# NVlabs/intrinsic3d

Hardware: AMD Instinct MI355X
Metric: Gauss-Newton iterations/s at the finest SDF level (higher is better)
Workload: dtype f32

## Files before the change

include/intrinsic3d_hip.h:

```cpp
#ifndef INTRINSIC3D_HIP_H
#define INTRINSIC3D_HIP_H
#include <stdint.h>
#ifdef __cplusplus
extern "C" {
#endif

typedef struct i3d_context i3d_context;

typedef enum {
    I3D_OK = 0,
    I3D_ERR_INVALID_ARGUMENT = 1,
    I3D_ERR_NO_DEVICE = 2,
    I3D_ERR_HIP = 3,
    I3D_ERR_STATE = 4,
    I3D_ERR_CAPACITY = 5,
    I3D_ERR_COMM = 6,
    I3D_ERR_IO = 7
} i3d_status;

int  i3d_create(int32_t device_ordinal, i3d_context** out);
void i3d_destroy(i3d_context* ctx);
const char* i3d_last_error(const i3d_context* ctx);
const char* i3d_version(void);

// ... 222 lines not shown
int i3d_timing_get_work_ex(i3d_context* ctx, double* ms, int64_t* launches, double* slow_ms , int64_t* slow_launches );
const char* i3d_kernel_name(int32_t k);
int i3d_problem_sizes(i3d_context* ctx, int64_t out[6]);

int i3d_debug_assemble(i3d_context* ctx, const i3d_optimizer_config* cfg, int32_t iteration, int32_t* slots_out);
int64_t i3d_debug_map_order(const int32_t* keys, int64_t n, int32_t mode, int32_t* order);
int i3d_debug_flags(i3d_context* ctx, uint8_t* flags );
int i3d_debug_eg_rows(i3d_context* ctx, int32_t* frame , float* weight ,
                      float* residual , float* jac );
int i3d_debug_reg_rows(i3d_context* ctx, uint8_t* has_er , uint8_t* has_es , float* ea_weight );
int i3d_debug_neighbors(i3d_context* ctx, int32_t* nbr );
int i3d_debug_normal_eq(i3d_context* ctx, double* gradient, double* jtj_diag, double* cost);
int i3d_debug_jtj_apply(i3d_context* ctx, const double* x, double* y);
int i3d_debug_counters(i3d_context* ctx, int64_t* stream_syncs);
int i3d_debug_ladder_stats(i3d_context* ctx, int64_t* out6);
int i3d_debug_cull_stats(i3d_context* ctx, int64_t* pairs, int64_t* culled);

#ifdef __cplusplus
}
#endif
#endif
```

intrinsic3d_amd/binding.py:

```python
from __future__ import annotations

import ctypes as C
import os

import numpy as np

_HERE = os.path.dirname(os.path.abspath(__file__))
LIB_PATH = os.environ.get("I3D_LIB") or os.path.join(_HERE, "libintrinsic3d_hip.so")

K_NAMES = ["classify", "observe", "build", "eg_pass", "gather", "cost", "vector", "sh", "eg_aux", "comm", "eg_mr2", "eg_mr3"]


class OptimizerConfig(C.Structure):
    _fields_ = [("iterations", C.c_int32), ("lm_steps", C.c_int32),
                ("lambda_g", C.c_double), ("lambda_r0", C.c_double), ("lambda_r1", C.c_double),
                ("lambda_s0", C.c_double), ("lambda_s1", C.c_double), ("lambda_a", C.c_double),
                ("fix_poses", C.c_int32), ("fix_intrinsics", C.c_int32), ("fix_distortion", C.c_int32),
                ("occlusion_distance", C.c_float), ("num_observations", C.c_int32),
                ("thres_shell", C.c_double), ("grid_level", C.c_int32), ("rgbd_level", C.c_int32),
                ("pcg_fixed_iterations", C.c_int32), ("verbose", C.c_int32), ("carry_trust_radius", C.c_int32), ("fix_sdf", C.c_int32)]


class IterationStats(C.Structure):
    _fields_ = [("rows", C.c_int64 * 4), ("weight_sum", C.c_double * 4), ("type_weight", C.c_double * 4),
# ... 77 lines not shown
           "i3d_set_frames", "i3d_set_frames_rgbd", "i3d_get_frame_image", "i3d_resize_depth", "i3d_set_camera", "i3d_get_camera", "i3d_set_voxel_sh", "i3d_get_voxel_sh",
           "i3d_optimizer_config_default", "i3d_optimize", "i3d_optimize_host", "i3d_estimate_sh",
           "i3d_set_grid_from_tsdf_records", "i3d_recompute_colors", "i3d_clear_outside_thin_shell", "i3d_upsample", "i3d_grid_info",
           "i3d_export_grid", "i3d_refine",
           "i3d_tsdf_read_header", "i3d_tsdf_read_records", "i3d_tsdf_write", "i3d_sbr_write", "i3d_sbr_read", "i3d_write_poses",
           "i3d_write_intrinsics", "i3d_read_intrinsics", "i3d_config_load_yaml", "i3d_yaml_get",
           "i3d_extract_mesh", "i3d_get_mesh", "i3d_render_view", "i3d_track_desc_default", "i3d_track_frame", "i3d_export_mesh_ply", "i3d_write_ply", "i3d_mc_tables", "i3d_visualization_colors",
           "i3d_png_info", "i3d_png_decode", "i3d_pose_mat_to_vec6", "i3d_sensor_open", "i3d_sensor_open_yaml", "i3d_sensor_close", "i3d_sensor_info", "i3d_sensor_color",
           "i3d_sensor_depth", "i3d_sensor_pose", "i3d_sensor_set_pose", "i3d_sensor_set_pose_vec6", "i3d_sensor_save_poses",
           "i3d_mesh_remove_loose_components", "i3d_keyframes_load", "i3d_keyframes_save", "i3d_keyframes_select", "i3d_blur_score", "i3d_init_frames_from_sensor",
           "i3d_fusion_create", "i3d_fusion_destroy", "i3d_fusion_last_error", "i3d_fusion_integrate", "i3d_fusion_finish", "i3d_fusion_info", "i3d_fusion_get",
           "i3d_fusion_save", "i3d_fusion_render", "i3d_fusion_track", "i3d_shard_need", "i3d_comm_stats",
           "i3d_comm_unique_id", "i3d_comm_init", "i3d_comm_sim_create", "i3d_comm_sim_destroy", "i3d_comm_init_sim", "i3d_shard_plan", "i3d_shard_vec_index",
           "i3d_comm_transport", "i3d_timing_enable", "i3d_timing_select", "i3d_timing_get", "i3d_timing_get_work", "i3d_timing_get_work_ex", "i3d_kernel_name", "i3d_problem_sizes",
           "i3d_debug_assemble", "i3d_debug_map_order", "i3d_debug_flags", "i3d_debug_eg_rows", "i3d_debug_reg_rows", "i3d_debug_neighbors",
           "i3d_debug_normal_eq", "i3d_debug_jtj_apply", "i3d_debug_counters", "i3d_debug_cull_stats", "i3d_debug_ladder_stats", "i3d_debug_track_sums"]

_lib = None


def load():
    global _lib
    if _lib is not None:
        return _lib
    if not os.path.exists(LIB_PATH):
        raise RuntimeError(f"{LIB_PATH} is missing: build it with `make -C intrinsic3d_amd/csrc` "
                           "(or __graft_entry__.build()); the product path has no CPU fallback")
    L = C.CDLL(LIB_PATH)
    vp, i32, i64, f32, f64 = C.c_void_p, C.c_int32, C.c_int64, C.c_float, C.c_double
    L.i3d_create.restype = i32; L.i3d_create.argtypes = [i32, C.POINTER(vp)]
    L.i3d_destroy.argtypes = [vp]
# ... 30 lines not shown
    L.i3d_timing_get.restype = i32; L.i3d_timing_get.argtypes = [vp, vp, vp, i32]
    L.i3d_timing_get_work.restype = i32; L.i3d_timing_get_work.argtypes = [vp, vp, vp]
    L.i3d_timing_get_work_ex.restype = i32; L.i3d_timing_get_work_ex.argtypes = [vp, vp, vp, vp, vp]
    L.i3d_kernel_name.restype = C.c_char_p; L.i3d_kernel_name.argtypes = [i32]
    L.i3d_comm_transport.restype = C.c_char_p; L.i3d_comm_transport.argtypes = [vp]
    L.i3d_problem_sizes.restype = i32; L.i3d_problem_sizes.argtypes = [vp, vp]
    L.i3d_debug_assemble.restype = i32; L.i3d_debug_assemble.argtypes = [vp, C.POINTER(OptimizerConfig), i32, C.POINTER(i32)]
    L.i3d_debug_flags.restype = i32; L.i3d_debug_flags.argtypes = [vp, vp]
    L.i3d_debug_eg_rows.restype = i32; L.i3d_debug_eg_rows.argtypes = [vp, vp, vp, vp, vp]
    L.i3d_debug_reg_rows.restype = i32; L.i3d_debug_reg_rows.argtypes = [vp, vp, vp, vp]
    L.i3d_debug_neighbors.restype = i32; L.i3d_debug_neighbors.argtypes = [vp, vp]
    L.i3d_debug_normal_eq.restype = i32; L.i3d_debug_normal_eq.argtypes = [vp, vp, vp, C.POINTER(f64)]
    L.i3d_debug_jtj_apply.restype = i32; L.i3d_debug_jtj_apply.argtypes = [vp, vp, vp]
    L.i3d_debug_counters.restype = i32; L.i3d_debug_counters.argtypes = [vp, vp]
    L.i3d_debug_ladder_stats.restype = i32; L.i3d_debug_ladder_stats.argtypes = [vp, vp]
    L.i3d_debug_cull_stats.restype = i32; L.i3d_debug_cull_stats.argtypes = [vp, vp, vp]
    L.i3d_set_grid_from_tsdf_records.restype = i32; L.i3d_set_grid_from_tsdf_records.argtypes = [vp, f32, i64, vp, vp, vp, vp]
    L.i3d_recompute_colors.restype = i32; L.i3d_recompute_colors.argtypes = [vp, f32, i32]
    L.i3d_clear_outside_thin_shell.restype = i32; L.i3d_clear_outside_thin_shell.argtypes = [vp, f64, C.POINTER(i64)]
    L.i3d_upsample.restype = i32; L.i3d_upsample.argtypes = [vp, C.POINTER(i64)]
    L.i3d_grid_info.restype = i32; L.i3d_grid_info.argtypes = [vp, C.POINTER(i64), C.POINTER(f32), C.POINTER(f32)]
    L.i3d_export_grid.restype = i32; L.i3d_export_grid.argtypes = [vp, vp, vp, vp, vp, vp, vp]
    L.i3d_refine.restype = i32; L.i3d_refine.argtypes = [vp, C.POINTER(RefineConfig), C.POINTER(OptimizerConfig), REFINE_CALLBACK, vp]
    u64 = C.c_uint64; cp = C.c_char_p
    L.i3d_tsdf_read_header.restype = i32; L.i3d_tsdf_read_header.argtypes = [cp, C.POINTER(f32), C.POINTER(f32), C.POINTER(f32), C.POINTER(u64), C.POINTER(f32)]
    L.i3d_tsdf_read_records.restype = i32; L.i3d_tsdf_read_records.argtypes = [cp, u64, vp, vp, vp, vp]
    L.i3d_tsdf_write.restype = i32; L.i3d_tsdf_write.argtypes = [cp, f32, f32, f32, f32, u64, vp, vp, vp, vp]
    L.i3d_sbr_write.restype = i32; L.i3d_sbr_write.argtypes = [cp, f32, f32, f32, f32, u64, vp, vp, vp, vp, vp, vp]
    L.i3d_sbr_read.restype = i32; L.i3d_sbr_read.argtypes = [cp, u64, vp, vp, vp, vp, vp, vp]
    L.i3d_write_poses.restype = i32; L.i3d_write_poses.argtypes = [cp, i32, vp, vp]
# ... 354 lines not shown
        NP = 2 * self.N + 6 * self.K + 9
        g = np.zeros(NP); d = np.zeros(NP); cost = C.c_double(0)
        self._check(self.L.i3d_debug_normal_eq(self.h, _p(g), _p(d), C.byref(cost)), "i3d_debug_normal_eq")
        return g, d, cost.value

    def debug_counters(self):
        n = C.c_int64(0)
        self._check(self.L.i3d_debug_counters(self.h, C.byref(n)), "i3d_debug_counters")
        return {"stream_syncs": int(n.value)}

    def debug_ladder_stats(self):
        a = (C.c_int64 * 6)()
        self._check(self.L.i3d_debug_ladder_stats(self.h, a), "i3d_debug_ladder_stats")
        return {"batches": int(a[0]), "row_streams": int(a[1]), "system_passes": int(a[2]), "resyncs": int(a[3]), "unused_systems": int(a[4]), "depth": int(a[5])}

    def debug_cull_stats(self):
        a = C.c_int64(0); b = C.c_int64(0)
        self._check(self.L.i3d_debug_cull_stats(self.h, C.byref(a), C.byref(b)), "i3d_debug_cull_stats")
        return int(a.value), int(b.value)

    def debug_jtj_apply(self, x):
        x = np.ascontiguousarray(x, np.float64); y = np.zeros_like(x)
        self._check(self.L.i3d_debug_jtj_apply(self.h, _p(x), _p(y)), "i3d_debug_jtj_apply")
        return y


def shard_need(A, world, anbr, active):
    anbr = np.ascontiguousarray(anbr, np.int32); active = np.ascontiguousarray(active, np.uint8); need = np.zeros(A, np.uint64)
    rc = load().i3d_shard_need(int(A), int(world), _p(anbr), _p(active), _p(need))
    if rc != 0:
# ... 329 lines not shown
```

intrinsic3d_amd/csrc/device/kernels.hpp:

```cpp
#pragma once
#include "common.hpp"
#include "p2p_device.hpp"

namespace i3d {

struct HashTable { unsigned long long* keys; int* vals; unsigned int mask; };
void launch_sort_keys(hipStream_t st, int N, const int* keys_xyz , unsigned long long* sort_keys, int* iota);
void launch_permute_grid(hipStream_t st, int N, const int* perm, const int* keys_xyz, const double* sdf, const double* sdf_ref,
                         const double* alb, const float* w, const uint8_t* rgb,
                         int* cx, int* cy, int* cz, int* rank, double* sdf0, double* x_sdf, double* x_alb, float* f_sdf, float* f_alb,
                         float* weight, uchar4* color);
void launch_hash_build(hipStream_t st, int N, const int* cx, const int* cy, const int* cz, HashTable t);
void launch_nbr_build(hipStream_t st, int N, const int* cx, const int* cy, const int* cz, HashTable t, int* nbr);
void launch_classify(hipStream_t st, GridView g, OptParams p, int* active_flag);
void launch_compact(hipStream_t st, int N, const int* active_flag, const int* active_scan, const uint8_t* flags, int* aidx, int* alist, uint8_t* aflags);
void launch_partition_blocks(hipStream_t st, GridView g, int A, int* alist, uint8_t* aflags, int* aidx);
void launch_group_rows(hipStream_t st, int A, const uint8_t* nrows, int* gmax);
void launch_anbr(hipStream_t st, int N, int A, int Acap, const int* alist, const int* nbr, const int* aidx, int* anbr);
void launch_scatter_sh(hipStream_t st, int N, const int* rank, const double* sh_visit , float* sh );
void launch_gather_visit(hipStream_t st, int N, const int* rank, const double* x_sdf, const double* x_alb, double* out_sdf, double* out_alb);
void launch_update_fields(hipStream_t st, int N, const int* rank, const double* sdf_ref, const double* alb, const uint8_t* rgb,
                          double* x_sdf, double* x_alb, float* f_sdf, float* f_alb, uchar4* color);

void launch_observe(hipStream_t st, GridView g, RowView r, OptParams p, const FrameConst* frames, const unsigned* cull_mask = nullptr, bool prefilter = false);
// ... 81 lines not shown
int    tile_plan_hmax();
inline int tile_plan_hmax_of(int T) { return T == 1024 ? 2048 : 1536; }
inline int tile_plan_tiles_of(int A, int T) { return (A + T - 1) / T; }
size_t tile_plan_temp_bytes(int ntiles);
hipError_t launch_tile_plan(hipStream_t st, RowView r, TilePlan t, void* temp, size_t temp_bytes);
void launch_eaw_sym(hipStream_t st, RowView r, TilePlan t, const int* cflag );
int  launch_eg_tile(hipStream_t st, RowView r, OptParams p, const float* u, TilePlan t, double* shared, float* qacc, double* pq_partials ,
                    const PcgState* state, float* cam_partials = nullptr, int cam_stride = 0);
void launch_ext_offsets(hipStream_t st, int n, const int* ext_e, int A, int* ext_off);
void eg_tile_launch_shape(const TilePlan& t, int K, int& blocks, int& tiles_per_block);

struct LadVec;
int  eg_tile_mr_max_systems(int K);
int  launch_eg_tile_mr(hipStream_t st, RowView r, OptParams p, TilePlan t, int nsys, const int* sys, const float* u0, float* qacc0, float* qh0, double* pq0 , float* cam0, int cam_stride,
                       const PcgState* st0 , const LadVec& lv);

struct ShardArgs {
    P2PDev pd; RimLists rim; int seq;
    int n_slice_partials;
    int n_rim_wg;
    const float* zb; float* pb; float* ub; const float* cmb; int chunk;
};
struct LadVec {
    size_t vec;
    size_t qh;
    size_t cam;
    size_t part;
    size_t mblk;
    size_t tail;
    int sysid[LADDER_MAX];
// ... 59 lines not shown
```

intrinsic3d_amd/csrc/device/tile_pass_mr.hip:

```cpp
#include <cstring>
#include <algorithm>
#include <vector>
#include <cstdlib>
#include "kernels.hpp"
#include "reduce_device.hpp"
#include "wave_ops.hpp"
#include "tile_device.hpp"

namespace i3d {

constexpr int MR_T = 512, MR_HMAX = 1536, MR_NWV = MR_T / 64, MR_TC = 32;

template <int NB> struct MrConst {
    static constexpr int T = MR_T, HMAX = MR_HMAX, NW = MR_NWV, TC = MR_TC, NSLOT = T + HMAX + 1;
    static constexpr int CAMW = (NW * 9 + 3) & ~3, VSTR = NW * TC * 6;
    static constexpr int O_U = 0, UB = (2 * NSLOT + 3) & ~3;
    static constexpr int O_TR = O_U + NB * UB, TRB = (T + 4 + 3) & ~3;
    static constexpr int D_FLAG = O_TR + NB * TRB, D_CAM9W = D_FLAG + 4, D_TAG = D_CAM9W + NB * CAMW, D_VAL = D_TAG + NW * TC;
    static constexpr int O_LIST = D_VAL + NB * VSTR, O_C = O_LIST + 2 * HMAX, O_OFFS = O_C + 12 * T, O_PQ = O_OFFS + (((HMAX + 4) / 2 + 3) & ~3), D0 = O_PQ + NB * 2 * T;
};
struct MrLayout { int o_upose, o_ui, SK; size_t bytes; };
static __host__ __device__ inline MrLayout mr_layout(int D0, int NB, int K) {
    const int rs = (6 * K) | 1;
    MrLayout L;
    L.o_upose = (rs + 9 + 3) & ~3; L.o_ui = (L.o_upose + 6 * K + 3) & ~3; L.SK = L.o_ui + 12;
// ... 61 lines not shown
constexpr int MR_NPH = 12;
__device__ unsigned long long g_mr_phase[3][MR_NPH + 2];
#define PH_DECL unsigned long long ph_[MR_NPH] = {0, 0, 0, 0, 0, 0, 0, 0, 0, 0, 0, 0}; unsigned long long ph_t_ = __builtin_amdgcn_s_memtime(); unsigned ph_tiles_ = 0
#define PH(k) do { const unsigned long long t_ = __builtin_amdgcn_s_memtime(); ph_[k] += t_ - ph_t_; ph_t_ = t_; } while (0)
#define PH_TILE ++ph_tiles_
#define PH_FLUSH(NBv) do { if ((threadIdx.x & 63u) == 0u) { for (int k_ = 0; k_ < MR_NPH; ++k_) atomicAdd(&g_mr_phase[(NBv) - 1][k_], ph_[k_]); atomicAdd(&g_mr_phase[(NBv) - 1][MR_NPH], (unsigned long long)ph_tiles_); atomicAdd(&g_mr_phase[(NBv) - 1][MR_NPH + 1], 1ull); } } while (0)
#else
#define PH_DECL
#define PH(k)
#define PH_TILE
#define PH_FLUSH(NBv)
#endif
#ifdef I3D_MR_BLOCKTIME
__device__ unsigned long long g_mr_blk[3][1024], g_mr_blk_n[3][1024];
#define BT_DECL const unsigned long long bt0_ = __builtin_amdgcn_s_memtime()
#define BT_FLUSH(NBv) do { if (threadIdx.x == 0u && blockIdx.x < 1024u) { atomicAdd(&g_mr_blk[(NBv) - 1][blockIdx.x], __builtin_amdgcn_s_memtime() - bt0_); atomicAdd(&g_mr_blk_n[(NBv) - 1][blockIdx.x], 1ull); } } while (0)
#else
#define BT_DECL
#define BT_FLUSH(NBv)
#endif

struct MrArgs {
    const float* u0; float* qacc0; float* qh0; double* pq0 ; float* cam0;
    const PcgState* st0;
    size_t vec, qh, cam, part;
    int sys[3];
};

template <int NB, bool GHOSTS>
__global__ void __launch_bounds__(MR_T, 2) k_eg_tile_mr(RowView r, OptParams p, MrArgs m, const unsigned* __restrict__ lnbr, const float* __restrict__ eaw_sym, const int* __restrict__ halo_idx,
                                                        const int* __restrict__ halo_cnt, int tiles_per_block, int ntl, int cam_stride, const int* __restrict__ gmaxv,
                                                        const unsigned short* __restrict__ hp_off, const unsigned short* __restrict__ hp_src,
                                                        int tile_first, int n_own, const int* __restrict__ ghost_list) {
    constexpr int T = MR_T, HMAX = MR_HMAX, NW = MR_NWV, TC = MR_TC, ZSLOT = T + HMAX, NCOL = 12, HPCAP = 4 * HMAX, NQH = HMAX / T;
    bool alive[NB];
    {
        bool any = false;
#pragma unroll
        for (int b = 0; b < NB; ++b) { alive[b] = m.st0[2 * m.sys[b]].done == 0; any = any || alive[b]; }
        if (!any) return;
    }
    extern __shared__ float lds[];
    const int K = p.K; const size_t Acap = r.Acap; const int A = r.A, chunk = r.chunk;
    const int nshared = 6 * K + 9, rs = (6 * K) | 1;
    using MC = MrConst<NB>;
    constexpr int D_FLAG = MC::D_FLAG, D_CAM9W = MC::D_CAM9W, CAMW = MC::CAMW, D_TAG = MC::D_TAG, D_VAL = MC::D_VAL, D0 = MC::D0;
    const MrLayout L = mr_layout(D0, NB, K);
    const int SB = L.SK, o_upose = L.o_upose, o_ui = L.o_ui;
#define SYS(b) (D0 + (b) * SB)
#define U_S(b) (MC::O_U + (b) * MC::UB)
#define U_A(b) (MC::O_U + (b) * MC::UB + MC::NSLOT)
#define TR_L(b) (MC::O_TR + (b) * MC::TRB)
#define C_L (MC::O_C)
#define hp_list reinterpret_cast<unsigned short*>(lds + MC::O_LIST)
// ... 7 lines not shown
        for (int e = i; e < rs + 9; e += T) lds[SYS(b) + e] = 0.0f;
        for (int e = i; e < 6 * K; e += T) lds[SYS(b) + o_upose + e] = ub[tail + e];
        if (i < 12) lds[SYS(b) + o_ui + i] = i < 9 ? ub[tail + 6 * K + i] : 0.0f;
    }
    if (lane < TC) lds[D_TAG + wave * TC + lane] = __int_as_float(-1);
    const int o_tag = D_TAG + wave * TC, o_val = D_VAL + wave * (TC * 6 * NB);
    for (int e = lane; e < TC * 6 * NB; e += 64) lds[o_val + e] = 0.0f;
    int tcount = 0;
    float cam9[NB][9];
#define PQ_L(b) reinterpret_cast<double*>(lds + MC::O_PQ + (b) * 2 * T)
#pragma unroll
    for (int b = 0; b < NB; ++b) { PQ_L(b)[i] = 0.0;
#pragma unroll
        for (int q = 0; q < 9; ++q) cam9[b][q] = 0.0f; }
    const float tw0 = p.type_wf[0], tw1 = p.type_wf[1], tw2 = p.type_wf[2], tw3 = p.type_wf[3];
    const int tile0 = blockIdx.x * tiles_per_block;
    const int tk_end = min(tile0 + tiles_per_block, ntl);

    int tile = 0, base = 0, a = 0, H = 0, nr_ld = 0; bool in = false, owned = false; size_t ac = 0;
    uint8_t fl = 0, rf_ld = 0; unsigned ln[5]; RowBlock rwA, rwB;
    float us[NB], ua[NB], hs[NB][NQH], ha[NB][NQH];
    auto tile_of = [&](int tk) { return (GHOSTS && tk >= n_own) ? ghost_list[tk - n_own] : (GHOSTS ? tile_first + tk : tk); };
    constexpr int NQL = (HPCAP / 8 + T - 1) / T, NQO = (HMAX + 1 + T - 1) / T;
    uint4 hpl[NQL]; unsigned short hpo[NQO];
    const char* wave_rows = reinterpret_cast<const char*>(r.rows);
    int gm = 0;
    const unsigned lane16 = (threadIdx.x & 63u) * 16u;
    auto load_block = [&](RowBlock& rw, int k) {
        const __amdgpu_buffer_rsrc_t rsrc = __builtin_amdgcn_make_buffer_rsrc((void*)wave_rows, 0, k < gm ? MAX_SLOTS * ROW_BLOCK_F4 * 16 : 0, 0x00020000);
#pragma unroll
        for (int q = 0; q < 7; ++q) { const v4u_b v = __builtin_amdgcn_raw_buffer_load_b128(rsrc, lane16, k * (ROW_BLOCK_F4 * 16) + q * 1024, 2 );
                                      rw.p[q] = make_float4(__uint_as_float(v.x), __uint_as_float(v.y), __uint_as_float(v.z), __uint_as_float(v.w)); }
        { const v2u_b t = __builtin_amdgcn_raw_buffer_load_b64(rsrc, lane16 >> 1, k * (ROW_BLOCK_F4 * 16) + 64 * ROW_PLANES * 16, 2); rw.j28 = __uint_as_float(t.x); rw.tag = (int)t.y; }
    };
    auto group_rows = [&](int tk) -> int {
        const int wa0 = tile_of(tk) * T + (int)(threadIdx.x & ~63u);
        const int grp = __builtin_amdgcn_readfirstlane(wa0 < A ? (wa0 >> 6) : -1);
        return grp >= 0 ? gmaxv[grp] : 0;
    };
    int he[NQH];
    auto issue_idx = [&](int tk) {
        tile = tile_of(tk); base = tile * T; a = base + i; in = a < A; ac = in ? (size_t)a : 0;
        owned = GHOSTS ? (a >= r.own0 && a < r.own1) : in;
        { const int wa0 = base + (int)(threadIdx.x & ~63u);
          const unsigned grp = (unsigned)__builtin_amdgcn_readfirstlane(wa0 < A ? (wa0 >> 6) : 0);
          wave_rows = reinterpret_cast<const char*>(r.rows + (size_t)grp * (size_t)(r.slots * ROW_BLOCK_F4)); }
        H = halo_cnt[tile];
#pragma unroll
// ... 238 lines not shown
    __syncthreads();
    for (int w = 0; w < NW; ++w) { if (wave == w) mr_table_merge<NB>(lds, o_tag, o_val, tcount, D0, SB); __syncthreads(); }
    if (threadIdx.x < 9) {
#pragma unroll
        for (int b = 0; b < NB; ++b) { float v = 0.0f; for (int w = 0; w < NW; ++w) v += lds[D_CAM9W + b * CAMW + w * 9 + threadIdx.x]; lds[SYS(b) + rs + threadIdx.x] = v; }
    }
    __syncthreads();
#pragma unroll
    for (int b = 0; b < NB; ++b) {
        if (!alive[b]) continue;
        float* const cam = m.cam0 + (size_t)m.sys[b] * m.cam;
        for (int q = threadIdx.x; q < nshared; q += T) {
            float v;
            if (q < 6 * K) { v = 0.0f; v += lds[SYS(b) + q]; }
            else v = lds[SYS(b) + rs + q - 6 * K];
            cam[(size_t)blockIdx.x * cam_stride + q] = v;
        }
    }
    if (m.pq0) {
#pragma unroll
        for (int b = 0; b < NB; ++b) { if (alive[b]) block_partial_d(PQ_L(b)[i], m.pq0 + (size_t)m.sys[b] * m.part, 1, 0); }
    }
    PH(11); PH_FLUSH(NB); BT_FLUSH(NB);
#undef SYS
#undef U_S
#undef U_A
#undef TR_L
#undef C_L
#undef hp_list
#undef hp_offs
#undef PQ_L
}

#ifdef I3D_MR_PHASES
static void mr_phase_report() {
    unsigned long long h[3][MR_NPH + 2];
    if (hipMemcpyFromSymbol(h, HIP_SYMBOL(g_mr_phase), sizeof(h)) != hipSuccess) return;
    static const char* name[MR_NPH] = {"prologue", "issue loads", "staging writes (gather wait)", "staging barrier", "regulariser rows + hoist", "row loop", "reverse slots / Ea weights",
// ... 27 lines not shown

int eg_tile_mr_max_systems(int K) {
    for (int nb = 3; nb >= 1; --nb) if (mr_lds_bytes(nb, K) <= I3D_LDS_LIMIT) return nb;
    return 0;
}

int launch_eg_tile_mr(hipStream_t st, RowView r, OptParams p, TilePlan t, int nsys, const int* sys, const float* u0, float* qacc0, float* qh0, double* pq0, float* cam0, int cam_stride,
                      const PcgState* st0, const LadVec& lv) {
    if (r.A <= 0 || nsys < 1 || nsys > 3 || t.T != MR_T || !t.hp_off || r.slots != 5) return 0;
    int blocks = 0, tiles_per_block = 0;
    eg_tile_launch_shape(t, p.K, blocks, tiles_per_block);
    if (blocks <= 0) return 0;
    const int ntl = t.ntiles_own + t.n_ghost;
    const bool gh = t.n_ghost > 0 || t.tile_first != 0 || r.own0 != 0 || r.own1 < r.A;
    MrArgs m; m.u0 = u0; m.qacc0 = qacc0; m.qh0 = qh0; m.pq0 = pq0; m.cam0 = cam0; m.st0 = st0; m.vec = lv.vec; m.qh = lv.qh; m.cam = lv.cam; m.part = lv.part;
    for (int b = 0; b < 3; ++b) m.sys[b] = sys[b < nsys ? b : nsys - 1];
    const size_t lds = mr_lds_bytes(nsys, p.K);
#define I3D_MR2(NB, GH) do { \
        if (!set_dynamic_lds((const void*)k_eg_tile_mr<NB, GH>, "k_eg_tile_mr", lds, p.K)) return 0; \
        k_eg_tile_mr<NB, GH><<<blocks, MR_T, lds, st>>>(r, p, m, t.lnbr, t.eaw_sym, t.halo_idx, t.halo_cnt, tiles_per_block, ntl, cam_stride, r.gmax, t.hp_off, t.hp_src, t.tile_first, t.ntiles_own, t.ghost_tiles); } while (0)
#define I3D_MR(NB) do { if (gh) I3D_MR2(NB, true); else I3D_MR2(NB, false); } while (0)
    if (nsys == 1) I3D_MR(1); else if (nsys == 2) I3D_MR(2); else I3D_MR(3);
#undef I3D_MR2
#undef I3D_MR
    return blocks;
}

}
```

intrinsic3d_amd/csrc/host/capi.cpp:

```cpp
#include <cstdlib>
#include "context.hpp"

using namespace i3d;

extern "C" {

int i3d_optimize(i3d_context* c, const i3d_optimizer_config* cfg, i3d_iteration_stats* stats) {
    if (!c || !cfg) return ctx_fail(c, I3D_ERR_INVALID_ARGUMENT, "i3d_optimize: null argument");
    return optimize(c, *cfg, stats);
}

int i3d_optimize_host(int32_t device_ordinal, const i3d_optimizer_config* cfg, const i3d_grid_view* grid,
                      double* sdf_refined_io, double* albedo_io, int32_t num_frames, int32_t levels, const int32_t* widths,
                      const int32_t* heights, const float* const* lum, const float* const* depth,
                      double* intr_io, double* dist_io, double* poses_io, const double* voxel_sh, i3d_iteration_stats* stats) {
    if (!cfg || !grid || !sdf_refined_io || !albedo_io || !intr_io || !dist_io || !poses_io || !voxel_sh) return I3D_ERR_INVALID_ARGUMENT;
    i3d_context* c = nullptr;
    int rc = i3d_create(device_ordinal, &c); if (rc) return rc;
    i3d_grid_view gv = *grid; gv.sdf_refined = sdf_refined_io; gv.albedo = albedo_io;
    rc = i3d_set_grid(c, &gv);
    if (!rc) rc = i3d_set_frames(c, num_frames, levels, widths, heights, lum, depth, nullptr);
    if (!rc) rc = i3d_set_camera(c, intr_io, dist_io, poses_io);
    if (!rc) rc = i3d_set_voxel_sh(c, voxel_sh);
    if (!rc) rc = i3d_optimize(c, cfg, stats);
// ... 156 lines not shown
int i3d_debug_jtj_apply(i3d_context* c, const double* x, double* y) {
    if (!c || !x || !y) return ctx_fail(c, I3D_ERR_INVALID_ARGUMENT, "i3d_debug_jtj_apply: null pointer");
    return jtj_apply_debug(c, x, y);
}
int i3d_debug_counters(i3d_context* c, int64_t* stream_syncs) {
    if (!c) return I3D_ERR_INVALID_ARGUMENT;
    if (stream_syncs) *stream_syncs = (int64_t)c->n_syncs;
    return I3D_OK;
}

int i3d_debug_ladder_stats(i3d_context* c, int64_t* out6) {
    if (!c || !out6) return I3D_ERR_INVALID_ARGUMENT;
    out6[0] = c->lad_batches; out6[1] = c->lad_streams; out6[2] = c->lad_system_passes; out6[3] = c->lad_resyncs; out6[4] = c->lad_wasted; out6[5] = c->ladder_max;
    return I3D_OK;
}

int i3d_debug_cull_stats(i3d_context* c, int64_t* pairs, int64_t* culled) {
    if (!c || !pairs || !culled) return I3D_ERR_INVALID_ARGUMENT;
    if (!c->cull_mask.p || c->nC <= 0) return ctx_fail(c, I3D_ERR_STATE, "i3d_debug_cull_stats: nothing assembled");
    const size_t ngroups = ((size_t)c->nC + 63) / 64, ncw = ((size_t)c->K + 31) / 32;
    *pairs = (int64_t)(ngroups * (size_t)c->K);
    if (!c->cull_on) { *culled = -1; return I3D_OK; }
    std::vector<unsigned> m(ngroups * ncw);
    CTX_HIP(c, hipSetDevice(c->device));
    CTX_HIP(c, hipMemcpy(m.data(), c->cull_mask.p, m.size() * sizeof(unsigned), hipMemcpyDeviceToHost));
    int64_t n = 0; for (unsigned w : m) n += __builtin_popcount(w);
    *culled = n;
    return I3D_OK;
}

// ... 2 lines not shown
```

intrinsic3d_amd/csrc/host/context.hpp:

```cpp
#pragma once
#include <functional>
#include <string>
#include <vector>
#include <cstring>
#include <cmath>
#include "../device/kernels.hpp"
#include "../device/render_kernels.hpp"
#include "../device/track_kernels.hpp"
#include "comm.hpp"
#include "../../../include/intrinsic3d_hip.h"

namespace i3d {

template <class T>
struct DevBuf {
    T* p = nullptr; size_t n = 0;
    DevBuf() = default;
    DevBuf(const DevBuf&) = delete; DevBuf& operator=(const DevBuf&) = delete;
    DevBuf(DevBuf&& o) noexcept : p(o.p), n(o.n) { o.p = nullptr; o.n = 0; }
    DevBuf& operator=(DevBuf&& o) noexcept { if (this != &o) { release(); p = o.p; n = o.n; o.p = nullptr; o.n = 0; } return *this; }
    ~DevBuf() { release(); }
    void release() { if (p) (void)hipFree(p); p = nullptr; n = 0; }
    hipError_t alloc(size_t count) {
        if (count <= n && p) return hipSuccess;
// ... 77 lines not shown
    i3d::DevBuf<float> aux_part;
    i3d::DevBuf<unsigned> tp_lnbr; i3d::DevBuf<int> tp_halo_idx, tp_halo_cnt, tp_iota, tp_ext_e, tp_ext_pos, tp_ext_off, tp_overflow; i3d::DevBuf<float> tp_qh, tp_eaw, cam_part;
    i3d::DevBuf<unsigned char> tp_temp; bool tile_ok = false;
    i3d::DevBuf<unsigned short> tp_hp_off, tp_hp_src; bool halo_pull = false;
    bool ladder_lists = false;
    bool mr1_serial = false;
    int ladder_max = 1;
    int ladder_hint = 0, ladder_hint_prev = 0;
    i3d::LadVec lad{};
    i3d::DevBuf<float> lad_vec;
    i3d::DevBuf<float> lad_qh, lad_cam, lad_mblk, lad_tail;
    i3d::DevBuf<double> lad_part;
    i3d::DevBuf<double> lad_red;
    i3d::DevBuf<i3d::PcgState> lad_st;
    long long lad_batches = 0, lad_streams = 0, lad_system_passes = 0, lad_resyncs = 0, lad_wasted = 0;
    double t_add_end = 0.0;
    bool deterministic = false;
    int tile_T = 0;
    int plan_T() const { return tile_T > 0 ? tile_T : i3d::tile_plan_T(); }
    i3d::TilePlan tile_plan() const {
        const int T = plan_T();
        const bool sh = comm && (comm->world > 1 || comm->force);
        const int t0 = sh ? own0 / T : 0, t1 = sh ? (own1 + T - 1) / T : i3d::tile_plan_tiles_of(A, T);
        return i3d::TilePlan{tp_lnbr.p, tp_eaw.p, tp_halo_idx.p, tp_halo_cnt.p, tp_iota.p, tp_ext_e.p, tp_ext_pos.p, tp_qh.p, tp_ext_off.p, tp_overflow.p, T, i3d::tile_plan_hmax_of(T), t0, t1 > t0 ? t1 - t0 : 0,
                             ghost_tiles.p, sh ? n_ghost_tiles : 0, deterministic ? 1 : 0, (halo_pull || ladder_lists) ? tp_hp_off.p : nullptr, (halo_pull || ladder_lists) ? tp_hp_src.p : nullptr, halo_pull ? 1 : 0};
    }

    i3d::DevBuf<float> v_mask, v_c, v_S, v_cm, v_D2, v_Minv, v_b, v_x, v_r, v_p, v_z, v_q, v_u, v_acc, v_tmp, v_qacc;
    i3d::DevBuf<float> Minv_blocks;
    i3d::DevBuf<double> d_shared, d_blocks, d_scal, d_xshared, d_xcshared;
// ... 50 lines not shown
```

intrinsic3d_amd/csrc/host/solver.cpp:

```cpp
#include "context.hpp"
#include <rocprim/rocprim.hpp>
#include <chrono>
#include <limits>
#include <algorithm>

namespace i3d {

#ifdef I3D_MR_PHASES
void mr_phase_report_now();
#endif
#ifdef I3D_MR_BLOCKTIME
void mr_blocktime_report_now();
#endif

static double now_s() { return std::chrono::duration<double>(std::chrono::steady_clock::now().time_since_epoch()).count(); }

static OptParams make_params(const i3d_context* c, const i3d_optimizer_config& cfg, const double* intr, const double* dist) {
    OptParams p; std::memset(&p, 0, sizeof(p));
    p.thres_shell = cfg.thres_shell; p.lambda_a = cfg.lambda_a; p.K = c->K; p.level = cfg.rgbd_level;
    p.pyr_scale = 1.0 / std::pow(2.0, cfg.rgbd_level);
    p.occlusion = cfg.occlusion_distance;
    p.use_er = (cfg.lambda_r0 > 0.0 && cfg.lambda_r1 > 0.0); p.use_es = (cfg.lambda_s0 > 0.0 && cfg.lambda_s1 > 0.0); p.use_ea = cfg.lambda_a > 0.0;
    for (int i = 0; i < 4; ++i) { p.intr[i] = intr[i]; p.cam_f[i] = (float)(intr[i] * p.pyr_scale); }
    bool dz = true;
// ... 564 lines not shown
static int pcg_solve_ladder(i3d_context* c, const i3d_optimizer_config& cfg, const OptParams& p, int B, const PcgState** finals, int* passes_out) {
    hipStream_t s = c->stream;
    const Layout L = layout_of(c);
    const int K = c->K; const size_t to = L.tail_off; const Seg2 own = L.own;
    RowView r = c->row_view(); TilePlan tp = c->tile_plan();
    LadVec lv = c->lad;
    float* const X0 = lad_vecp(c, LV_X); float* const R0 = lad_vecp(c, LV_R); float* const P0 = lad_vecp(c, LV_P); float* const Z0 = lad_vecp(c, LV_Z);
    float* const U0 = lad_vecp(c, LV_U); float* const Q0 = lad_vecp(c, LV_Q);
    PcgState* const st2 = c->lad_st.p;
    const int NSP = (L.NS + 3) & ~3;
    double* const step_part0 = c->lad_part.p; double* const pq_part0 = step_part0 + LAD_PART_STEP; double* const d2_part0 = pq_part0 + LAD_PART_PQ;
    const bool use_mr = [] { const char* e = std::getenv("I3D_LADDER_MR"); return !(e && e[0] == '0'); }();
    const bool mr1 = [] { const char* e = std::getenv("I3D_LADDER_MR1"); return e && e[0] == '1'; }();
    const int group_cap = [] { const char* e = std::getenv("I3D_LADDER_GROUP"); const int v = e ? std::atoi(e) : 3; return v < 1 ? 1 : (v > 3 ? 3 : v); }();
    const int mr_cap = std::min(group_cap, eg_tile_mr_max_systems(K));
    const bool mr_ok = use_mr && mr_cap >= 1 && tp.T == 512 && tp.hp_off != nullptr && r.slots == 5;
    const bool sh = sharded(c);
    double* const red4 = sh ? c->lad_red.p : nullptr;
    const int rstride = (int)lad_redop_stride(L.NS);
    double* const redop = sh ? c->lad_red.p + (size_t)LADDER_MAX * 4 : nullptr;
    { TimedScope t(c, I3D_K_VECTOR);
      for (int j = 0; j < B; ++j) { CTX_HIP(c, hipMemsetAsync(X0 + (size_t)j * lv.vec, 0, sizeof(float) * L.NP, s));
                                    CTX_HIP(c, hipMemcpyAsync(R0 + (size_t)j * lv.vec, c->v_b.p, sizeof(float) * L.NP, hipMemcpyDeviceToDevice, s)); }
      launch_pcg_init_lad(s, st2, B, cfg.pcg_fixed_iterations, 500, c->d_lm.p); }
    Step3Args a; std::memset(&a, 0, sizeof(a));
    auto c4 = [&](const float* v) { return reinterpret_cast<const float4*>(v + own.off0); };
    auto m4 = [&](float* v) { return reinterpret_cast<float4*>(v + own.off0); };
    a.nq = own.n >> 2; a.chunk4 = (int)((own.off1 - own.off0) >> 2);
    a.p = c4(P0); a.qacc = c4(Q0); a.x = m4(X0); a.r = m4(R0); a.b = c4(c->v_b.p); a.z = m4(Z0); a.cm = c4(c->v_cm.p); a.lm = c->d_lm.p;
    a.ext_off = tp.ext_off; a.ext_pos = tp.ext_pos; a.qh = reinterpret_cast<const float2*>(c->lad_qh.p); a.e0 = (int)own.off0;
// ... 1 lines not shown
    a.n_slice_wg = pcg_step3_slice_wgs(own.n, 0);
    a.sharded = 0; a.lad_sys = 0; a.redop = redop; a.redop_stride = rstride;
    a.K = K; a.fix_poses = p.fix_poses; a.fix_intr = p.fix_intr; a.fix_dist = p.fix_dist;
    a.cam_partials = c->lad_cam.p; a.n_cam = 0; a.cam_stride = NSP; a.Mblk = c->lad_mblk.p;
    a.tp = P0 + to; a.tx = X0 + to; a.tr = R0 + to; a.tb = c->v_b.p + to; a.tD2 = c->lad_tail.p; a.tz = Z0 + to; a.tS = c->v_S.p + to;
    a.step_partials = step_part0;
    std::vector<int> live(B); for (int j = 0; j < B; ++j) live[j] = j;
    auto set_slots = [&]() { for (int q = 0; q < LADDER_MAX; ++q) lv.sysid[q] = live[q < (int)live.size() ? q : (int)live.size() - 1]; };
    auto rows_apply = [&](int parity, bool with_dot) -> int {
        int n = 0; const int nl = (int)live.size();
        if (sh) { TimedScope t(c, I3D_K_COMM);
                  if (c->comm->push_halo_multi(U0, lv.vec, live.data(), nl, c->halo, s)) return -1; }
        if (mr_ok && (nl > 1 || mr1 || sh)) {
            const int groups = (nl + mr_cap - 1) / mr_cap;
            int at = 0;
            for (int g = 0; g < groups; ++g) {
                const int ng = (nl - at + (groups - g) - 1) / (groups - g);
                TimedScope t(c, ng == 1 ? I3D_K_EG_PASS : (ng == 2 ? I3D_K_EG_MR2 : I3D_K_EG_MR3));
                n = launch_eg_tile_mr(s, r, p, tp, ng, live.data() + at, U0, Q0, c->lad_qh.p, with_dot ? pq_part0 : nullptr, c->lad_cam.p, NSP, st2 + parity, lv);
                if (n <= 0) return -1;
                at += ng; ++c->lad_streams;
            }
        } else {
            for (int j : live) {
                TilePlan tj = tp; tj.qh = c->lad_qh.p + (size_t)j * lv.qh;
                TimedScope t(c, I3D_K_EG_PASS);
                n = launch_eg_tile(s, r, p, U0 + (size_t)j * lv.vec, tj, nullptr, Q0 + (size_t)j * lv.vec, with_dot ? pq_part0 + (size_t)j * lv.part : nullptr, st2 + 2 * j + parity,
                                   c->lad_cam.p + (size_t)j * lv.cam, NSP);
                ++c->lad_streams;
            }
        }
        c->lad_system_passes += nl;
        if (sh) {
            { TimedScope t(c, I3D_K_VECTOR); launch_lad_reduce_op(s, nl, c->lad_cam.p, n, NSP, L.NS, pq_part0, with_dot ? n : 0, d2_part0, with_dot ? a.n_d2 : 0, redop, rstride, lv); }
            if (allreduce(c, redop, (size_t)LADDER_MAX * rstride)) return -1;
        }
        return n;
    };
    auto step_sums = [&](int nl, int n_slice) -> int {
        if (!sh) return I3D_OK;
        { TimedScope t(c, I3D_K_VECTOR); launch_lad_reduce_step(s, nl, step_part0, n_slice, red4, lv); }
        return allreduce(c, red4, (size_t)LADDER_MAX * 4);
    };
    int n_step = 0;
    set_slots();
    { TimedScope t(c, I3D_K_VECTOR); a.cur = st2; n_step = launch_pcg_step3_lad(s, 0 , B, a, lv); }
    const int seq0 = c->pcg_seq;
// ... 278 lines not shown
```

Before: 41.75.

## Fuse two multi-RHS tile-pass groups into one paired kernel launch

When the live PCG ladder systems split into two groups (4-6 live systems, non-sharded), a single launch of a paired multi-RHS tile kernel now covers both groups, interleaving workgroups in blocks of 8 so each half handles one system group. This replaces two back-to-back kernel launches with one grid of twice the size, aiming to cut launch gaps and tail underutilisation. The row-buffer load cache policy (aux bits) also becomes a compile-time macro defaulting to 0 instead of 2, and per-block pq partials are written directly. Debug counters for live-system histograms and paired passes are added.

```diff
diff --git a/include/intrinsic3d_hip.h b/include/intrinsic3d_hip.h
--- a/include/intrinsic3d_hip.h
+++ b/include/intrinsic3d_hip.h
@@ -260,6 +260,7 @@
 int i3d_debug_jtj_apply(i3d_context* ctx, const double* x, double* y);
 int i3d_debug_counters(i3d_context* ctx, int64_t* stream_syncs);
 int i3d_debug_ladder_stats(i3d_context* ctx, int64_t* out6);
+int i3d_debug_ladder_passes(i3d_context* ctx, int64_t* out8);
 int i3d_debug_cull_stats(i3d_context* ctx, int64_t* pairs, int64_t* culled);
 
 #ifdef __cplusplus
diff --git a/intrinsic3d_amd/binding.py b/intrinsic3d_amd/binding.py
--- a/intrinsic3d_amd/binding.py
+++ b/intrinsic3d_amd/binding.py
@@ -115,7 +115,7 @@
            "i3d_comm_unique_id", "i3d_comm_init", "i3d_comm_sim_create", "i3d_comm_sim_destroy", "i3d_comm_init_sim", "i3d_shard_plan", "i3d_shard_vec_index",
            "i3d_comm_transport", "i3d_timing_enable", "i3d_timing_select", "i3d_timing_get", "i3d_timing_get_work", "i3d_timing_get_work_ex", "i3d_kernel_name", "i3d_problem_sizes",
            "i3d_debug_assemble", "i3d_debug_map_order", "i3d_debug_flags", "i3d_debug_eg_rows", "i3d_debug_reg_rows", "i3d_debug_neighbors",
-           "i3d_debug_normal_eq", "i3d_debug_jtj_apply", "i3d_debug_counters", "i3d_debug_cull_stats", "i3d_debug_ladder_stats", "i3d_debug_track_sums"]
+           "i3d_debug_normal_eq", "i3d_debug_jtj_apply", "i3d_debug_counters", "i3d_debug_cull_stats", "i3d_debug_ladder_stats", "i3d_debug_ladder_passes", "i3d_debug_track_sums"]
 
 _lib = None
 
@@ -176,6 +176,7 @@
     L.i3d_debug_jtj_apply.restype = i32; L.i3d_debug_jtj_apply.argtypes = [vp, vp, vp]
     L.i3d_debug_counters.restype = i32; L.i3d_debug_counters.argtypes = [vp, vp]
     L.i3d_debug_ladder_stats.restype = i32; L.i3d_debug_ladder_stats.argtypes = [vp, vp]
+    L.i3d_debug_ladder_passes.restype = i32; L.i3d_debug_ladder_passes.argtypes = [vp, vp]
     L.i3d_debug_cull_stats.restype = i32; L.i3d_debug_cull_stats.argtypes = [vp, vp, vp]
     L.i3d_set_grid_from_tsdf_records.restype = i32; L.i3d_set_grid_from_tsdf_records.argtypes = [vp, f32, i64, vp, vp, vp, vp]
     L.i3d_recompute_colors.restype = i32; L.i3d_recompute_colors.argtypes = [vp, f32, i32]
@@ -560,6 +561,11 @@
         self._check(self.L.i3d_debug_ladder_stats(self.h, a), "i3d_debug_ladder_stats")
         return {"batches": int(a[0]), "row_streams": int(a[1]), "system_passes": int(a[2]), "resyncs": int(a[3]), "unused_systems": int(a[4]), "depth": int(a[5])}
 
+    def debug_ladder_passes(self):
+        a = (C.c_int64 * 8)()
+        self._check(self.L.i3d_debug_ladder_passes(self.h, a), "i3d_debug_ladder_passes")
+        return {"live": [int(a[n]) for n in range(7)], "paired": int(a[7])}
+
     def debug_cull_stats(self):
         a = C.c_int64(0); b = C.c_int64(0)
         self._check(self.L.i3d_debug_cull_stats(self.h, C.byref(a), C.byref(b)), "i3d_debug_cull_stats")
diff --git a/intrinsic3d_amd/csrc/device/kernels.hpp b/intrinsic3d_amd/csrc/device/kernels.hpp
--- a/intrinsic3d_amd/csrc/device/kernels.hpp
+++ b/intrinsic3d_amd/csrc/device/kernels.hpp
@@ -119,6 +119,8 @@
 int  eg_tile_mr_max_systems(int K);
 int  launch_eg_tile_mr(hipStream_t st, RowView r, OptParams p, TilePlan t, int nsys, const int* sys, const float* u0, float* qacc0, float* qh0, double* pq0 , float* cam0, int cam_stride,
                        const PcgState* st0 , const LadVec& lv);
+int  launch_eg_tile_mr_pair(hipStream_t st, RowView r, OptParams p, TilePlan t, int na, int nb, const int* sys, const float* u0, float* qacc0, float* qh0, double* pq0 , float* cam0,
+                            int cam_stride, const PcgState* st0, const LadVec& lv);
 
 struct ShardArgs {
     P2PDev pd; RimLists rim; int seq;
diff --git a/intrinsic3d_amd/csrc/device/tile_pass_mr.hip b/intrinsic3d_amd/csrc/device/tile_pass_mr.hip
--- a/intrinsic3d_amd/csrc/device/tile_pass_mr.hip
+++ b/intrinsic3d_amd/csrc/device/tile_pass_mr.hip
@@ -9,6 +9,9 @@
 
 namespace i3d {
 
+#ifndef I3D_MR_ROW_AUX
+#define I3D_MR_ROW_AUX 0
+#endif
 constexpr int MR_T = 512, MR_HMAX = 1536, MR_NWV = MR_T / 64, MR_TC = 32;
 
 template <int NB> struct MrConst {
@@ -100,10 +103,10 @@
 #ifdef I3D_MR_BLOCKTIME
 __device__ unsigned long long g_mr_blk[3][1024], g_mr_blk_n[3][1024];
 #define BT_DECL const unsigned long long bt0_ = __builtin_amdgcn_s_memtime()
-#define BT_FLUSH(NBv) do { if (threadIdx.x == 0u && blockIdx.x < 1024u) { atomicAdd(&g_mr_blk[(NBv) - 1][blockIdx.x], __builtin_amdgcn_s_memtime() - bt0_); atomicAdd(&g_mr_blk_n[(NBv) - 1][blockIdx.x], 1ull); } } while (0)
+#define BT_FLUSH(NBv, wgv) do { if (threadIdx.x == 0u && (unsigned)(wgv) < 1024u) { atomicAdd(&g_mr_blk[(NBv) - 1][wgv], __builtin_amdgcn_s_memtime() - bt0_); atomicAdd(&g_mr_blk_n[(NBv) - 1][wgv], 1ull); } } while (0)
 #else
 #define BT_DECL
-#define BT_FLUSH(NBv)
+#define BT_FLUSH(NBv, wgv)
 #endif
 
 struct MrArgs {
@@ -111,19 +114,24 @@
     const PcgState* st0;
     size_t vec, qh, cam, part;
     int sys[3];
+    int sysb[3]; int nsysb; int blocks;
 };
 
-template <int NB, bool GHOSTS>
+template <int NB, bool GHOSTS, bool PAIR = false>
 __global__ void __launch_bounds__(MR_T, 2) k_eg_tile_mr(RowView r, OptParams p, MrArgs m, const unsigned* __restrict__ lnbr, const float* __restrict__ eaw_sym, const int* __restrict__ halo_idx,
                                                         const int* __restrict__ halo_cnt, int tiles_per_block, int ntl, int cam_stride, const int* __restrict__ gmaxv,
                                                         const unsigned short* __restrict__ hp_off, const unsigned short* __restrict__ hp_src,
                                                         int tile_first, int n_own, const int* __restrict__ ghost_list) {
     constexpr int T = MR_T, HMAX = MR_HMAX, NW = MR_NWV, TC = MR_TC, ZSLOT = T + HMAX, NCOL = 12, HPCAP = 4 * HMAX, NQH = HMAX / T;
+    const int w_id = (int)blockIdx.x;
+    const int group = PAIR ? (w_id >> 3) & 1 : 0, wg = PAIR ? (w_id >> 4) * 8 + (w_id & 7) : w_id;
+    if (PAIR && wg >= m.blocks) return;
+    if (PAIR && group) { m.sys[0] = m.sysb[0]; m.sys[1] = m.sysb[1]; m.sys[2] = m.sysb[2]; }
     bool alive[NB];
     {
         bool any = false;
 #pragma unroll
-        for (int b = 0; b < NB; ++b) { alive[b] = m.st0[2 * m.sys[b]].done == 0; any = any || alive[b]; }
+        for (int b = 0; b < NB; ++b) { alive[b] = m.st0[2 * m.sys[b]].done == 0 && !(PAIR && group && b >= m.nsysb); any = any || alive[b]; }
         if (!any) return;
     }
     extern __shared__ float lds[];
@@ -161,7 +169,7 @@
 #pragma unroll
         for (int q = 0; q < 9; ++q) cam9[b][q] = 0.0f; }
     const float tw0 = p.type_wf[0], tw1 = p.type_wf[1], tw2 = p.type_wf[2], tw3 = p.type_wf[3];
-    const int tile0 = blockIdx.x * tiles_per_block;
+    const int tile0 = wg * tiles_per_block;
     const int tk_end = min(tile0 + tiles_per_block, ntl);
 
     int tile = 0, base = 0, a = 0, H = 0, nr_ld = 0; bool in = false, owned = false; size_t ac = 0;
@@ -176,9 +184,9 @@
     auto load_block = [&](RowBlock& rw, int k) {
         const __amdgpu_buffer_rsrc_t rsrc = __builtin_amdgcn_make_buffer_rsrc((void*)wave_rows, 0, k < gm ? MAX_SLOTS * ROW_BLOCK_F4 * 16 : 0, 0x00020000);
 #pragma unroll
-        for (int q = 0; q < 7; ++q) { const v4u_b v = __builtin_amdgcn_raw_buffer_load_b128(rsrc, lane16, k * (ROW_BLOCK_F4 * 16) + q * 1024, 2 );
+        for (int q = 0; q < 7; ++q) { const v4u_b v = __builtin_amdgcn_raw_buffer_load_b128(rsrc, lane16, k * (ROW_BLOCK_F4 * 16) + q * 1024, I3D_MR_ROW_AUX);
                                       rw.p[q] = make_float4(__uint_as_float(v.x), __uint_as_float(v.y), __uint_as_float(v.z), __uint_as_float(v.w)); }
-        { const v2u_b t = __builtin_amdgcn_raw_buffer_load_b64(rsrc, lane16 >> 1, k * (ROW_BLOCK_F4 * 16) + 64 * ROW_PLANES * 16, 2); rw.j28 = __uint_as_float(t.x); rw.tag = (int)t.y; }
+        { const v2u_b t = __builtin_amdgcn_raw_buffer_load_b64(rsrc, lane16 >> 1, k * (ROW_BLOCK_F4 * 16) + 64 * ROW_PLANES * 16, I3D_MR_ROW_AUX); rw.j28 = __uint_as_float(t.x); rw.tag = (int)t.y; }
     };
     auto group_rows = [&](int tk) -> int {
         const int wa0 = tile_of(tk) * T + (int)(threadIdx.x & ~63u);
@@ -447,14 +455,14 @@
             float v;
             if (q < 6 * K) { v = 0.0f; v += lds[SYS(b) + q]; }
             else v = lds[SYS(b) + rs + q - 6 * K];
-            cam[(size_t)blockIdx.x * cam_stride + q] = v;
+            cam[(size_t)wg * cam_stride + q] = v;
         }
     }
     if (m.pq0) {
 #pragma unroll
-        for (int b = 0; b < NB; ++b) { if (alive[b]) block_partial_d(PQ_L(b)[i], m.pq0 + (size_t)m.sys[b] * m.part, 1, 0); }
-    }
-    PH(11); PH_FLUSH(NB); BT_FLUSH(NB);
+        for (int b = 0; b < NB; ++b) { if (alive[b]) { const double t = block_sum_d(PQ_L(b)[i]); if (threadIdx.x == 0) (m.pq0 + (size_t)m.sys[b] * m.part)[wg] = t; } }
+    }
+    PH(11); PH_FLUSH(NB); BT_FLUSH(NB, wg);
 #undef SYS
 #undef U_S
 #undef U_A
@@ -512,7 +520,8 @@
     const int ntl = t.ntiles_own + t.n_ghost;
     const bool gh = t.n_ghost > 0 || t.tile_first != 0 || r.own0 != 0 || r.own1 < r.A;
     MrArgs m; m.u0 = u0; m.qacc0 = qacc0; m.qh0 = qh0; m.pq0 = pq0; m.cam0 = cam0; m.st0 = st0; m.vec = lv.vec; m.qh = lv.qh; m.cam = lv.cam; m.part = lv.part;
-    for (int b = 0; b < 3; ++b) m.sys[b] = sys[b < nsys ? b : nsys - 1];
+    for (int b = 0; b < 3; ++b) { m.sys[b] = sys[b < nsys ? b : nsys - 1]; m.sysb[b] = m.sys[b]; }
+    m.nsysb = nsys; m.blocks = 0;
     const size_t lds = mr_lds_bytes(nsys, p.K);
 #define I3D_MR2(NB, GH) do { \
         if (!set_dynamic_lds((const void*)k_eg_tile_mr<NB, GH>, "k_eg_tile_mr", lds, p.K)) return 0; \
@@ -524,4 +533,25 @@
     return blocks;
 }
 
-}
+int launch_eg_tile_mr_pair(hipStream_t st, RowView r, OptParams p, TilePlan t, int na, int nb, const int* sys, const float* u0, float* qacc0, float* qh0, double* pq0, float* cam0, int cam_stride,
+                           const PcgState* st0, const LadVec& lv) {
+    if (r.A <= 0 || na > 3 || nb < 2 || nb > na || t.T != MR_T || !t.hp_off || r.slots != 5) return 0;
+    if (t.n_ghost > 0 || t.tile_first != 0 || r.own0 != 0 || r.own1 < r.A) return 0;
+    int blocks = 0, tiles_per_block = 0;
+    eg_tile_launch_shape(t, p.K, blocks, tiles_per_block);
+    if (blocks <= 0) return 0;
+    const int ntl = t.ntiles_own;
+    MrArgs m; m.u0 = u0; m.qacc0 = qacc0; m.qh0 = qh0; m.pq0 = pq0; m.cam0 = cam0; m.st0 = st0; m.vec = lv.vec; m.qh = lv.qh; m.cam = lv.cam; m.part = lv.part;
+    for (int b = 0; b < 3; ++b) { m.sys[b] = sys[b < na ? b : na - 1]; m.sysb[b] = sys[na + (b < nb ? b : nb - 1)]; }
+    m.nsysb = nb; m.blocks = blocks;
+    const size_t lds = mr_lds_bytes(na, p.K);
+    const int grid = 2 * ((blocks + 7) & ~7);
+#define I3D_MRP(NB) do { \
+        if (!set_dynamic_lds((const void*)k_eg_tile_mr<NB, false, true>, "k_eg_tile_mr (paired)", lds, p.K)) return 0; \
+        k_eg_tile_mr<NB, false, true><<<grid, MR_T, lds, st>>>(r, p, m, t.lnbr, t.eaw_sym, t.halo_idx, t.halo_cnt, tiles_per_block, ntl, cam_stride, r.gmax, t.hp_off, t.hp_src, 0, ntl, nullptr); } while (0)
+    if (na == 3) I3D_MRP(3); else I3D_MRP(2);
+#undef I3D_MRP
+    return blocks;
+}
+
+}
diff --git a/intrinsic3d_amd/csrc/host/capi.cpp b/intrinsic3d_amd/csrc/host/capi.cpp
--- a/intrinsic3d_amd/csrc/host/capi.cpp
+++ b/intrinsic3d_amd/csrc/host/capi.cpp
@@ -194,6 +194,12 @@
     out6[0] = c->lad_batches; out6[1] = c->lad_streams; out6[2] = c->lad_system_passes; out6[3] = c->lad_resyncs; out6[4] = c->lad_wasted; out6[5] = c->ladder_max;
     return I3D_OK;
 }
+int i3d_debug_ladder_passes(i3d_context* c, int64_t* out8) {
+    if (!c || !out8) return I3D_ERR_INVALID_ARGUMENT;
+    for (int n = 0; n < 7; ++n) out8[n] = c->lad_pass_live[n];
+    out8[7] = c->lad_paired;
+    return I3D_OK;
+}
 
 int i3d_debug_cull_stats(i3d_context* c, int64_t* pairs, int64_t* culled) {
     if (!c || !pairs || !culled) return I3D_ERR_INVALID_ARGUMENT;
diff --git a/intrinsic3d_amd/csrc/host/context.hpp b/intrinsic3d_amd/csrc/host/context.hpp
--- a/intrinsic3d_amd/csrc/host/context.hpp
+++ b/intrinsic3d_amd/csrc/host/context.hpp
@@ -115,6 +115,7 @@
     i3d::DevBuf<double> lad_red;
     i3d::DevBuf<i3d::PcgState> lad_st;
     long long lad_batches = 0, lad_streams = 0, lad_system_passes = 0, lad_resyncs = 0, lad_wasted = 0;
+    long long lad_pass_live[7] = {0, 0, 0, 0, 0, 0, 0}, lad_paired = 0;
     double t_add_end = 0.0;
     bool deterministic = false;
     int tile_T = 0;
diff --git a/intrinsic3d_amd/csrc/host/solver.cpp b/intrinsic3d_amd/csrc/host/solver.cpp
--- a/intrinsic3d_amd/csrc/host/solver.cpp
+++ b/intrinsic3d_amd/csrc/host/solver.cpp
@@ -602,6 +602,7 @@
     const bool mr1 = [] { const char* e = std::getenv("I3D_LADDER_MR1"); return e && e[0] == '1'; }();
     const int group_cap = [] { const char* e = std::getenv("I3D_LADDER_GROUP"); const int v = e ? std::atoi(e) : 3; return v < 1 ? 1 : (v > 3 ? 3 : v); }();
     const int mr_cap = std::min(group_cap, eg_tile_mr_max_systems(K));
+    const bool pair = [] { const char* e = std::getenv("I3D_LADDER_PAIR"); return !(e && e[0] == '0'); }();
     const bool mr_ok = use_mr && mr_cap >= 1 && tp.T == 512 && tp.hp_off != nullptr && r.slots == 5;
     const bool sh = sharded(c);
     double* const red4 = sh ? c->lad_red.p : nullptr;
@@ -633,7 +634,13 @@
         if (mr_ok && (nl > 1 || mr1 || sh)) {
             const int groups = (nl + mr_cap - 1) / mr_cap;
             int at = 0;
-            for (int g = 0; g < groups; ++g) {
+            if (groups == 2 && pair && !sh && nl - (nl + 1) / 2 >= 2) {
+                const int na = (nl + 1) / 2;
+                TimedScope t(c, na == 2 ? I3D_K_EG_MR2 : I3D_K_EG_MR3);
+                n = launch_eg_tile_mr_pair(s, r, p, tp, na, nl - na, live.data(), U0, Q0, c->lad_qh.p, with_dot ? pq_part0 : nullptr, c->lad_cam.p, NSP, st2 + parity, lv);
+                if (n > 0) { at = nl; ++c->lad_streams; ++c->lad_paired; }
+            }
+            for (int g = 0; g < groups && at < nl; ++g) {
                 const int ng = (nl - at + (groups - g) - 1) / (groups - g);
                 TimedScope t(c, ng == 1 ? I3D_K_EG_PASS : (ng == 2 ? I3D_K_EG_MR2 : I3D_K_EG_MR3));
                 n = launch_eg_tile_mr(s, r, p, tp, ng, live.data() + at, U0, Q0, c->lad_qh.p, with_dot ? pq_part0 : nullptr, c->lad_cam.p, NSP, st2 + parity, lv);
@@ -649,7 +656,7 @@
                 ++c->lad_streams;
             }
         }
-        c->lad_system_passes += nl;
+        c->lad_system_passes += nl; ++c->lad_pass_live[nl < 6 ? nl : 6];
         if (sh) {
             { TimedScope t(c, I3D_K_VECTOR); launch_lad_reduce_op(s, nl, c->lad_cam.p, n, NSP, L.NS, pq_part0, with_dot ? n : 0, d2_part0, with_dot ? a.n_d2 : 0, redop, rstride, lv); }
             if (allreduce(c, redop, (size_t)LADDER_MAX * rstride)) return -1;
```

Result: faster. 43.84, median of 6 (+5.0%).
